# valeoai/PAFUSE

Hardware: AMD Instinct MI355X
Metric: hypotheses/sec through DDIM loop (H3WB 133-kp, P=20, T=10) (higher is better)
Workload: dtype bf16x3 (every fp32 GEMM operand as the exact sum of three bf16 slices, six bf16 MFMA products per fp32-equivalent product, fp32 accumulate; activations, LayerNorm, softmax, attention and everything in memory fp32; the residual stream stored centred on its row means)

## Files before the change

pafuse_amd/csrc/kernels.hpp:

```cpp
#pragma once
#include <hip/hip_runtime.h>
#include <stdint.h>

#include <utility>

namespace pafuse {

typedef float f32x16 __attribute__((ext_vector_type(16)));
typedef float f32x4 __attribute__((ext_vector_type(4)));

constexpr int BK = 32;
constexpr int LDK = 36;

typedef __bf16 bf16x8 __attribute__((ext_vector_type(8)));
__device__ __forceinline__ bf16x8 to_bf16x8(const f32x4 lo, const f32x4 hi) {
    bf16x8 v;
#pragma unroll
    for (int i = 0; i < 4; ++i) v[i] = (__bf16)lo[i], v[4 + i] = (__bf16)hi[i];
    return v;
}

#ifdef PAFUSE_MFMA_K8
typedef __bf16 bf16x4_t __attribute__((ext_vector_type(4)));
typedef short s16x4_t __attribute__((ext_vector_type(4)));
// ... 1254 lines not shown
                    } else {
                        asm volatile("s_waitcnt lgkmcnt(3)" : "+v"(wf[g & 1][0]), "+v"(wf[g & 1][1]), "+v"(wf[g & 1][2]));
                    }
                } else {
                    asm volatile("s_waitcnt lgkmcnt(0)" : "+v"(wf[g & 1][0]), "+v"(wf[g & 1][1]), "+v"(wf[g & 1][2]));
                }
                const u32x4(&w)[3] = wf[g & 1];
                auto mm = [&](int wi, int ai) {
                    PAFUSE_PIN_ACC(acc[nt]);
                    acc[nt] = mfma_bf16_k16(__builtin_bit_cast(bf16x8, w[wi]), __builtin_bit_cast(bf16x8, cur[ai]), acc[nt]);
                };
                auto pins = [&]() {
    #pragma unroll
                    for (int q = q0; q < q1; ++q) PAFUSE_PIN_PAIR(sp[q]);
                };
                pins();
                mm(0, 2);
                {
                    constexpr int PER = (CNT + NG - 1) / NG, j0 = g * PER, j1 = (g + 1) * PER < CNT ? (g + 1) * PER : CNT;
                    if constexpr (j0 < j1 && ABL < 2) {
                        asm volatile("" ::: "memory");
                        if (refill) {
    #pragma unroll
                            for (int j = j0; j < j1; ++j) issue_piece(kn, stn, j);
                        }
                        asm volatile("" ::: "memory");
                    }
                }
    #pragma unroll
                for (int q = q0; q < q1; ++q) sp[q].template stage<0>();
                pins();
                mm(2, 0);
    #pragma unroll
                for (int q = q0; q < q1; ++q) sp[q].template stage<1>();
                pins();
                mm(1, 1);
    #pragma unroll
                for (int q = q0; q < q1; ++q) sp[q].template stage<2>();
                pins();
                mm(0, 1);
    #pragma unroll
                for (int q = q0; q < q1; ++q) sp[q].template stage<3>();
                pins();
                mm(1, 0);
    #pragma unroll
                for (int q = q0; q < q1; ++q) {
                    sp[q].template stage<4>();
                    nxt[0][q] = sp[q].s0, nxt[1][q] = sp[q].s1, nxt[2][q] = sp[q].s2;
                }
                pins();
                mm(0, 0);
                if constexpr (g == NT - 1 && ABL < 3 && NS2 == 2) cur[0] = nxt[0], cur[1] = nxt[1], cur[2] = nxt[2];
                if constexpr (g == NT - 1 && ABL >= 3 && NS2 == 2) {
    #pragma unroll
                    for (int q = 0; q < 4; ++q)
                        cur[0][q] = cur[2][q] = __builtin_bit_cast(uint32_t, sp[q].x0), cur[1][q] = __builtin_bit_cast(uint32_t, sp[q].x1);
                }
            });
    #undef PAFUSE_PIN_ACC
    #undef PAFUSE_PIN_PAIR
            __builtin_amdgcn_s_setprio(0);
        }
    }
    PAFUSE_STAMP(1);
    __syncthreads();
    constexpr int VEC = EPI == EPI_BIAS ? 0 : (7 * BM * WN + 3) / 4 * 4;
    if constexpr (VEC > 0) {
        static_assert((size_t)(VEC + 5 * BN) * sizeof(float) <= (size_t)NSTAGE * T::STAGE_BYTES, "epilogue vectors must fit the ring");
        const float* const src[5] = {p.bias, p.post_w, p.post_b, p.next_w, p.next_b};
#pragma unroll
        for (int v = 0; v < 5; ++v)
            if (src[v])
                for (int i = tid; i < BN / 4; i += T::NTHR)
                    *reinterpret_cast<f32x4*>(smem + VEC + v * BN + 4 * i) = *reinterpret_cast<const f32x4*>(src[v] + n0 + 4 * i);
        __syncthreads();
    }
    if constexpr (ABL == 4) {
        float sacc = 0.f;
#pragma unroll
        for (int nt = 0; nt < NT; ++nt)
#pragma unroll
            for (int i = 0; i < 16; ++i) sacc += acc[nt][i];
        if (sacc == 123.456f) p.out[0] = sacc;
        return;
    }
    if constexpr (EPI == EPI_ROWLN && SLAB) {
        constexpr size_t RINGF = (size_t)NSTAGE * T::STAGE_BYTES / sizeof(float);
        constexpr auto need = [](int nth) { return (size_t)VEC + 5 * BN + (size_t)NW * 32 * (32 * nth + 4); };
        constexpr int NTH = (NT % 2 == 0 && need(2) <= RINGF) ? 2 : 1;
        static_assert(need(NTH) <= RINGF, "epilogue scratch must fit the ring");
        epilogue_rows_h<WN, NT, BM, NW, NTH, false, 2>(acc, p, m0, n0, wm, wn, r, h, wave, lane, smem, 1.0f);
    } else {
        epilogue_row_per_lane<WN, NT, BM, EPI, VEC>(acc, p, m0, n0, wm, wn, r, h, smem);
    }
}

template <int WM, int WN, int NT, int EPI, int NSTAGE, int MINW, int ABL = 0, int BKC = 32>
__global__ void __launch_bounds__(WM* WN * 64, MINW) gemm_dma_kernel(const GemmParams p) {
    PAFUSE_XQ_GUARD();
    extern __shared__ __attribute__((aligned(16))) float smem[];
    gemm_dma_tile<WM, WN, NT, EPI, NSTAGE, ABL, BKC>(p, blockIdx.x, gridDim.x, smem);
}

constexpr int GROUP_MAX = 4;
struct GroupedGemmParams {
    GemmParams p[GROUP_MAX];
    int first[GROUP_MAX + 1];
    int n;
};

template <int EPI>
__global__ void __launch_bounds__(256, 2) grouped_rowln_kernel(const GroupedGemmParams g) {
    PAFUSE_XQ_GUARD();
    extern __shared__ __attribute__((aligned(16))) float smem[];
    const int b = blockIdx.x;
    int s = 0;
#pragma unroll
    for (int i = 1; i < GROUP_MAX; ++i)
        if (i < g.n && b >= g.first[i]) s = i;
    const GemmParams& p = g.p[s];
    const int lb = b - g.first[s], nb = g.first[s + 1] - g.first[s];
    switch (p.N) {
        case 384: gemm_dma_tile<2, 2, 6, EPI, 2, 0, 16, false>(p, lb, nb, smem); break;
        case 256: gemm_dma_tile<2, 2, 4, EPI, 2, 0, 16, false>(p, lb, nb, smem); break;
        case 224: gemm_dma_tile<4, 1, 7, EPI, 2, 0, 16, false>(p, lb, nb, smem); break;
        default: break;
    }
}

struct AttnParams {
    const float* qkv;
    float* o;
    uint8_t* o_h;
    int64_t nseq;
    int L, C, heads, d;
    int64_t group, group_stride, seq_stride, tok_stride;
    float scale;
};

template <int ITEMS>
__device__ __forceinline__ void attn_item(int64_t i, int64_t nseq, int heads, int64_t& seq, int& head) {
    if (nseq % 8 == 0 && ((nseq / 8) * heads) % ITEMS == 0) {
        const int64_t blk = i / ITEMS;
        const int lo = (int)(blk % 8);
        const int64_t u = (blk / 8) * ITEMS + (i % ITEMS);
        head = (int)(u % heads);
        seq = (u / heads) * 8 + lo;
    } else {
        seq = i / heads;
        head = (int)(i % heads);
    }
}

template <int LP, int DP, int NW>
__global__ void __launch_bounds__(NW * 64) attn_kernel(const AttnParams p) {
    PAFUSE_XQ_GUARD();
    constexpr int QT = LP / 16, KT = LP / 16, CT = DP / 16, SD = DP / 16, ITEMS = NW / QT, LDV = DP + 4;
    constexpr int NTHR = NW * 64, C4 = DP / 4;
    static_assert(NW % QT == 0, "waves must be a multiple of the query tiles");
    extern __shared__ __attribute__((aligned(16))) float smem[];
    float* Ks = smem;
    float* Vs = smem + ITEMS * LP * LDV;
    const int tid = threadIdx.x, lane = tid & 63, wave = tid >> 6;
    const int64_t nitems = p.nseq * p.heads;
    const int C3 = 3 * p.C;

    const int il = wave / QT, qt = wave % QT;
    const int64_t item = (int64_t)blockIdx.x * ITEMS + il;
    const bool mine = item < nitems;
    int64_t seq = 0;
    int head = 0;
    if (mine) attn_item<ITEMS>(item, p.nseq, p.heads, seq, head);
    const int64_t base = (seq / p.group) * p.group_stride + (seq % p.group) * p.seq_stride;
    const int l15 = lane & 15, g = lane >> 4;
    f32x4 qf[SD];
    {
        const int q = qt * 16 + l15;
#pragma unroll
        for (int s = 0; s < SD; ++s) {
            qf[s] = f32x4{0.f, 0.f, 0.f, 0.f};
            if (mine && q < p.L && 16 * s + 4 * g < p.d)
                qf[s] = *reinterpret_cast<const f32x4*>(p.qkv + (base + q * p.tok_stride) * C3 + head * p.d + 16 * s +
                                                        4 * g);
        }
    }
    for (int sl = 0; sl < ITEMS; ++sl) {
        const int64_t it2 = (int64_t)blockIdx.x * ITEMS + sl;
        const bool ok = it2 < nitems;
        int64_t seq2 = 0;
        int head2 = 0;
        if (ok) attn_item<ITEMS>(it2, p.nseq, p.heads, seq2, head2);
        const int64_t base2 = (seq2 / p.group) * p.group_stride + (seq2 % p.group) * p.seq_stride;
        for (int idx = tid; idx < LP * C4; idx += NTHR) {
            const int t = idx / C4, c4 = idx % C4;
            f32x4 kv = {0.f, 0.f, 0.f, 0.f}, vv = {0.f, 0.f, 0.f, 0.f};
            if (ok && t < p.L && c4 * 4 < p.d) {
                const float* src = p.qkv + (base2 + t * p.tok_stride) * C3 + head2 * p.d + c4 * 4;
                kv = *reinterpret_cast<const f32x4*>(src + p.C);
                vv = *reinterpret_cast<const f32x4*>(src + 2 * p.C);
            }
            *reinterpret_cast<f32x4*>(Ks + (sl * LP + t) * LDV + c4 * 4) = kv;
            *reinterpret_cast<f32x4*>(Vs + (sl * LP + t) * LDV + c4 * 4) = vv;
        }
    }
    __syncthreads();
    if (!mine) return;
    const float* Kb = Ks + il * LP * LDV;
    const float* Vb = Vs + il * LP * LDV;
    f32x4 sc[KT];
#pragma unroll
    for (int kt = 0; kt < KT; ++kt) sc[kt] = f32x4{0.f, 0.f, 0.f, 0.f};
#pragma unroll
    for (int s = 0; s < SD; ++s) {
        f32x4 kf[KT];
#pragma unroll
        for (int kt = 0; kt < KT; ++kt)
            kf[kt] = *reinterpret_cast<const f32x4*>(Kb + (kt * 16 + l15) * LDV + 16 * s + 4 * g);
#pragma unroll
        for (int j = 0; j < 4; ++j)
#pragma unroll
            for (int kt = 0; kt < KT; ++kt)
                sc[kt] = __builtin_amdgcn_mfma_f32_16x16x4f32(kf[kt][j], qf[s][j], sc[kt], 0, 0, 0);
    }
    float mx = -INFINITY;
#pragma unroll
    for (int kt = 0; kt < KT; ++kt)
#pragma unroll
        for (int reg = 0; reg < 4; ++reg) {
            const int key = kt * 16 + 4 * g + reg;
            const float v = key < p.L ? sc[kt][reg] * p.scale : -INFINITY;
            sc[kt][reg] = v;
            mx = fmaxf(mx, v);
        }
    mx = fmaxf(mx, __shfl_xor(mx, 16));
    mx = fmaxf(mx, __shfl_xor(mx, 32));
    float sum = 0.f;
#pragma unroll
    for (int kt = 0; kt < KT; ++kt)
#pragma unroll
        for (int reg = 0; reg < 4; ++reg) {
            const float e = __builtin_amdgcn_exp2f((sc[kt][reg] - mx) * 1.44269504088896340736f);
            sc[kt][reg] = e;
            sum += e;
        }
    sum += __shfl_xor(sum, 16);
    sum += __shfl_xor(sum, 32);
    const float inv = 1.0f / sum;
#pragma unroll
    for (int kt = 0; kt < KT; ++kt)
#pragma unroll
        for (int reg = 0; reg < 4; ++reg) sc[kt][reg] *= inv;

    f32x4 oc[CT];
#pragma unroll
    for (int ct = 0; ct < CT; ++ct) oc[ct] = f32x4{0.f, 0.f, 0.f, 0.f};
#pragma unroll
    for (int kt = 0; kt < KT; ++kt)
#pragma unroll
        for (int reg = 0; reg < 4; ++reg) {
            const float* vrow = Vb + (kt * 16 + 4 * g + reg) * LDV + l15;
#pragma unroll
            for (int ct = 0; ct < CT; ++ct)
                oc[ct] = __builtin_amdgcn_mfma_f32_16x16x4f32(vrow[ct * 16], sc[kt][reg], oc[ct], 0, 0, 0);
        }
    const int q = qt * 16 + l15;
    if (q < p.L) {
        if (p.o_h) {
            uint8_t* const hrow = p.o_h + (base + q * p.tok_stride) * p.C * 4;
#pragma unroll
            for (int ct = 0; ct < CT; ++ct)
                if (ct * 16 + 4 * g < p.d) {
                    const int c = head * p.d + ct * 16 + 4 * g;
                    hsplit_store4(hrow + (c >> 3) * 32, c & 4, oc[ct]);
                }
            return;
        }
        float* orow = p.o + (base + q * p.tok_stride) * p.C + head * p.d + 4 * g;
#pragma unroll
        for (int ct = 0; ct < CT; ++ct)
            if (ct * 16 + 4 * g < p.d) *reinterpret_cast<f32x4*>(orow + ct * 16) = oc[ct];
    }
}

constexpr int ATTN_LONG_LP = 256;
template <int DP>
__global__ void __launch_bounds__(1024) attn_long_kernel(const AttnParams p) {
    PAFUSE_XQ_GUARD();
    constexpr int LP = ATTN_LONG_LP, T = LP / 16, SD = DP / 16, CT = DP / 16, LDV = DP + 4, C4 = DP / 4;
    extern __shared__ __attribute__((aligned(16))) float smem[];
    float* Ks = smem;
    float* Vs = smem + LP * LDV;
    const int tid = threadIdx.x, lane = tid & 63, w = tid >> 6, l15 = lane & 15, g = lane >> 4;
    int64_t seq;
    int head;
    attn_item<1>((int64_t)blockIdx.x, p.nseq, p.heads, seq, head);
    const int64_t base = (seq / p.group) * p.group_stride + (seq % p.group) * p.seq_stride;
    const int C3 = 3 * p.C, nt = (p.L + 15) / 16;
    f32x4 qf[SD];
    {
        const int q = 16 * w + l15;
#pragma unroll
        for (int s = 0; s < SD; ++s) {
            qf[s] = f32x4{0.f, 0.f, 0.f, 0.f};
            if (q < p.L && 16 * s + 4 * g < p.d)
                qf[s] = *reinterpret_cast<const f32x4*>(p.qkv + (base + (int64_t)q * p.tok_stride) * C3 + head * p.d + 16 * s + 4 * g);
        }
    }
    for (int idx = tid; idx < nt * 16 * C4; idx += 1024) {
        const int t = idx / C4, c4 = idx % C4;
        f32x4 kv = {0.f, 0.f, 0.f, 0.f}, vv = {0.f, 0.f, 0.f, 0.f};
        if (t < p.L && c4 * 4 < p.d) {
            const float* src = p.qkv + (base + (int64_t)t * p.tok_stride) * C3 + head * p.d + c4 * 4;
            kv = *reinterpret_cast<const f32x4*>(src + p.C);
            vv = *reinterpret_cast<const f32x4*>(src + 2 * p.C);
        }
        *reinterpret_cast<f32x4*>(Ks + t * LDV + c4 * 4) = kv;
        *reinterpret_cast<f32x4*>(Vs + t * LDV + c4 * 4) = vv;
    }
    __syncthreads();
    if (w >= nt) return;
    f32x4 sc[T];
#pragma unroll
    for (int kt = 0; kt < T; ++kt) {
        sc[kt] = f32x4{0.f, 0.f, 0.f, 0.f};
        if (kt < nt) {
#pragma unroll
            for (int s = 0; s < SD; ++s) {
                const f32x4 kf = *reinterpret_cast<const f32x4*>(Ks + (kt * 16 + l15) * LDV + 16 * s + 4 * g);
#pragma unroll
                for (int j = 0; j < 4; ++j) sc[kt] = __builtin_amdgcn_mfma_f32_16x16x4f32(kf[j], qf[s][j], sc[kt], 0, 0, 0);
            }
        }
    }
    float mx = -INFINITY;
#pragma unroll
    for (int kt = 0; kt < T; ++kt)
#pragma unroll
        for (int reg = 0; reg < 4; ++reg) {
            const float v = kt * 16 + 4 * g + reg < p.L ? sc[kt][reg] * p.scale : -INFINITY;
            sc[kt][reg] = v;
            mx = fmaxf(mx, v);
        }
    mx = fmaxf(mx, __shfl_xor(mx, 16));
    mx = fmaxf(mx, __shfl_xor(mx, 32));
    float sum = 0.f;
#pragma unroll
    for (int kt = 0; kt < T; ++kt)
#pragma unroll
        for (int reg = 0; reg < 4; ++reg) {
            const float e = __builtin_amdgcn_exp2f((sc[kt][reg] - mx) * 1.44269504088896340736f);
            sc[kt][reg] = e;
            sum += e;
        }
    sum += __shfl_xor(sum, 16);
    sum += __shfl_xor(sum, 32);
    const float inv = 1.0f / sum;
    f32x4 oc[CT];
#pragma unroll
    for (int ct = 0; ct < CT; ++ct) oc[ct] = f32x4{0.f, 0.f, 0.f, 0.f};
#pragma unroll
    for (int kt = 0; kt < T; ++kt)
        if (kt < nt) {
#pragma unroll
            for (int reg = 0; reg < 4; ++reg) {
                const float pr = sc[kt][reg] * inv;
                const float* vrow = Vs + (kt * 16 + 4 * g + reg) * LDV + l15;
#pragma unroll
                for (int ct = 0; ct < CT; ++ct) oc[ct] = __builtin_amdgcn_mfma_f32_16x16x4f32(vrow[ct * 16], pr, oc[ct], 0, 0, 0);
            }
        }
    const int q = 16 * w + l15;
    if (q < p.L) {
        float* orow = p.o + (base + (int64_t)q * p.tok_stride) * p.C + head * p.d + 4 * g;
#pragma unroll
        for (int ct = 0; ct < CT; ++ct)
            if (ct * 16 + 4 * g < p.d) *reinterpret_cast<f32x4*>(orow + ct * 16) = oc[ct];
    }
}

struct FqaParams {
    GemmParams g;
    float* o;
    int64_t nseq;
    int L, C, heads, d, nseq_tile;
    int64_t group, group_stride, seq_stride, tok_stride;
    float scale;
};

template <int LP, int DP>
struct FqaTile {
    static constexpr int NB = 3 * DP / 16, LDV = DP + 4, ROWS = 128 + (LP == 48 ? 4 : 0);
    static constexpr int STAGE_BYTES = Tile16<NB>::STAGE_BYTES, QKV_BYTES = 3 * ROWS * LDV * 4;
    static constexpr int LDS_BYTES = STAGE_BYTES > QKV_BYTES ? STAGE_BYTES : QKV_BYTES;
};

template <int LP, int DP>
__global__ void __launch_bounds__(256, 2) fqa_kernel(const FqaParams fp) {
    PAFUSE_XQ_GUARD();
    using FT = FqaTile<LP, DP>;
    constexpr int NB = FT::NB, LDV = FT::LDV, ROWS = FT::ROWS;
    using T = Tile16<NB>;
    constexpr int A_LD = T::A_LD, W_LD = T::W_LD, NTHR = T::NTHR;
    extern __shared__ __attribute__((aligned(16))) float smem[];
    const GemmParams& p = fp.g;
    uint8_t* const As = reinterpret_cast<uint8_t*>(smem);
    uint8_t* const Ws = As + T::A_BYTES;
    const int tid = threadIdx.x, lane = tid & 63, wave = tid >> 6;
    const int c = lane & 15, qd = lane >> 4;
    const int L = fp.L, NSEQ = fp.nseq_tile;
    const int64_t ntiles = (fp.nseq + NSEQ - 1) / NSEQ;
    const int xcd = blockIdx.x & 7, idx = blockIdx.x >> 3;
    const int64_t tile = (int64_t)(idx / fp.heads) * 8 + xcd;
    const int head = idx % fp.heads;
    if (tile >= ntiles) return;
    const int K = p.K, nk = K / 32;
    const int64_t seq0 = tile * NSEQ;
    const int64_t last_seq = fp.nseq - 1;
    auto token_of = [&](int r) -> int64_t {
        int sl = r / L, t = r - sl * L;
        if (sl >= NSEQ) sl = NSEQ - 1, t = L - 1;
        int64_t sq = seq0 + sl;
        if (sq > last_seq) sq = last_seq;
        return (sq / fp.group) * fp.group_stride + (sq % fp.group) * fp.seq_stride + t * fp.tok_stride;
    };

    const float* a_ptr[A_LD];
    int a_dst[A_LD];
#pragma unroll
    for (int i = 0; i < A_LD; ++i) {
        const int g = 2 * wave + (i >> 1), j = 4 * (i & 1) + qd;
        a_ptr[i] = p.A + token_of(16 * g + c) * K + 4 * j;
        a_dst[i] = g * 2048 + (j & 1) * 1024 + ((j >> 1) * 16 + c) * 16;
    }
// ... 3246 lines not shown
```

pafuse_amd/csrc/pafuse_hip.hip:

```cpp
#include "../../include/pafuse_hip.h"

#include <hip/hip_runtime.h>

#include <algorithm>
#include <cmath>
#include <cstdarg>
#include <cstdio>
#include <cstdlib>
#include <cstring>
#include <type_traits>

#include "kernels.hpp"
#include "hgemm.hpp"
#include "xgemm.hpp"
#include "sgemm.hpp"
#include "train_kernels.hpp"

using namespace pafuse;

namespace {

thread_local char g_err[512] = "";

int fail(int code, const char* fmt, ...) {
// ... 372 lines not shown
        if (p.N % 64 == 0) return launch_gemm<4, 1, 2, EPI_BIAS, 1, 4, 0, 2>(p, s);
    }
    if (p.M <= 0) return PAFUSE_OK;
    if (p.K % BK || p.N % 32 || p.K <= 0 || p.N <= 0)
        return fail(PAFUSE_E_SHAPE, "linear: N=%d K=%d must be positive multiples of 32", p.N, p.K);
    if ((p.out_act || p.dact_u) && ((p.N % 64 && !(p.mode == MODE_BF16X3 && p.wlayout == WLAYOUT_M16)) || mode_images(p.mode) || p.ln_in || p.act))
        return fail(PAFUSE_E_ARG, "linear: out_act / dact_u need N %% 64 == 0 and a plain fp32 or bf16x3 product");
    if (p.mode == MODE_F16X2) return hgemm_bias(p, s);
    if (p.mode == MODE_BF16X3_IMAGES) return xgemm_bias(p, s);
#ifdef PAFUSE_QKV_32X32
    p.wlayout = WLAYOUT_PLAIN;
#endif
#ifndef PAFUSE_NO_STRIP
    if (strip2_ok(p)) return strip2_bias(p, s);
#endif
    if (p.mode == MODE_BF16X3 && p.wlayout == WLAYOUT_M16) {
        if (p.N % 128 == 0) return launch_gemm16<8, 3>(p, s);
        if (p.N % 96 == 0) return launch_gemm16<6, 3>(p, s);
        if (p.N % 112 == 0) return launch_gemm16<7, 3>(p, s);
        if (p.N % 64 == 0) return launch_gemm16<4, 4>(p, s);
        return launch_gemm16<2, 4>(p, s);
    }
    if (p.mode == MODE_BF16X3) {
        if (p.N % 128 == 0 && p.M >= 4096) return launch_gemm<4, 1, 4, EPI_BIAS, 1, PAFUSE_FC1_MINW, 0, 2>(p, s);
        if (p.N % 64 == 0) return launch_gemm<4, 1, 2, EPI_BIAS, 1, 4, 0, 2>(p, s);
        if (p.N % 96 == 0) return launch_gemm<4, 1, 3, EPI_BIAS, 1, 1, 1, 2>(p, s);
        return launch_gemm<4, 1, 1, EPI_BIAS, 1, 1, 0, 2>(p, s);
    }
    if (p.mode != MODE_F32) {
        if (p.N % 64 == 0) return launch_gemm<4, 1, 2, EPI_BIAS, 1, 5, 0, 1>(p, s);
        if (p.N % 96 == 0) return launch_gemm<4, 1, 3, EPI_BIAS, 1, 1, 1, 1>(p, s);
        return launch_gemm<4, 1, 1, EPI_BIAS, 1, 1, 0, 1>(p, s);
    }
    if (p.N % 64 == 0) return launch_gemm<4, 1, 2, EPI_BIAS, 1, 5>(p, s);
    if (p.N % 96 == 0) return launch_gemm<4, 1, 3, EPI_BIAS, 1, 1, 1>(p, s);
    return launch_gemm<4, 1, 1, EPI_BIAS, 1>(p, s);
}

template <int EPI>
int gemm_rowln_as(const GemmParams& p0, hipStream_t s) {
    GemmParams p = p0;
    if (p.mode == MODE_BF16X3 && (debug_f32_mask() & 2)) p.mode = MODE_F32;
    if (p.M <= 0) return PAFUSE_OK;
    if (p.K % BK || p.K <= 0) return fail(PAFUSE_E_SHAPE, "rowln: K=%d must be a positive multiple of 32", p.K);
    if (p.mode == MODE_F16X2 || p.mode == MODE_BF16X3_IMAGES) {
        if constexpr (EPI == EPI_ROWLN) return p.mode == MODE_F16X2 ? hgemm_rowln(p, s) : xgemm_rowln(p, s);
        else return fail(PAFUSE_E_ARG, "training has no image-pipeline kernels");
    }
    if constexpr (EPI == EPI_ROWLN_TRAIN) {
        if (p.mode == MODE_BF16X3) {
            switch (p.N) {
                case 384: return launch_gemm_dma<2, 2, 6, EPI, 2, 2, 16>(p, s);
                case 256: return launch_gemm_dma<2, 2, 4, EPI, 2, 2, 16>(p, s);
                case 224: if (p.M >= 4096) return launch_gemm_dma<4, 1, 7, EPI, 2, 2, 16>(p, s); break;
                default: break;
            }
            p.mode = MODE_F32;
        }
    }
    if constexpr (EPI == EPI_ROWLN) {
        if (p.mode == MODE_BF16X3) {
            switch (p.N) {
                case 384: return launch_gemm_dma<2, 2, 6, EPI, 2, 2, 16>(p, s);
                case 256: return launch_gemm_dma<2, 2, 4, EPI, 2, 2, 16>(p, s);
                case 288: return launch_gemm_dma<2, 3, 3, EPI, 2, 2, 16>(p, s);
                case 224:
                    return p.M >= 4096 ? launch_gemm_dma<4, 1, 7, EPI, 2, 2, 16>(p, s) : launch_gemm_dma<2, 1, 7, EPI, 2, 2, 16>(p, s);
                case 128: return launch_gemm<1, 4, 1, EPI, 1, 1, 1, 2>(p, s);
                case 64: return launch_gemm<1, 2, 1, EPI, 1, 1, 1, 2>(p, s);
                default: break;
            }
        } else if (p.mode != MODE_F32) {
            switch (p.N) {
                case 384: return launch_gemm<1, 4, 3, EPI, 1, 1, 1, 1>(p, s);
                case 288: return launch_gemm<1, 3, 3, EPI, 1, 1, 1, 1>(p, s);
                case 256: return launch_gemm<2, 2, 4, EPI, 1, 2, 1, 1>(p, s);
                case 224: return launch_gemm<1, 7, 1, EPI, 1, 1, 1, 1>(p, s);
                case 128: return launch_gemm<1, 4, 1, EPI, 1, 1, 1, 1>(p, s);
                case 64: return launch_gemm<1, 2, 1, EPI, 1, 1, 1, 1>(p, s);
                default: break;
            }
        }
    }
    switch (p.N) {
        case 384: return launch_gemm<1, 4, 3, EPI, 1, 1, 1>(p, s);
        case 288: return launch_gemm<1, 3, 3, EPI, 1, 1, 1>(p, s);
        case 256: return launch_gemm<2, 2, 4, EPI, 1, 2, 1>(p, s);
        case 224: return launch_gemm<1, 7, 1, EPI, 1, 1, 1>(p, s);
        case 128: return launch_gemm<1, 4, 1, EPI, 1, 1, 1>(p, s);
        case 64: return launch_gemm<1, 2, 1, EPI, 1, 1, 1>(p, s);
        default: return fail(PAFUSE_E_SHAPE, "no whole-row kernel for channel width %d (have 64,128,224,256,288,384)", p.N);
    }
}

int gemm_rowln(const GemmParams& p, hipStream_t s) { return gemm_rowln_as<EPI_ROWLN>(p, s); }
int gemm_rowln_train(const GemmParams& p, hipStream_t s) { return gemm_rowln_as<EPI_ROWLN_TRAIN>(p, s); }

bool group_ok_rowln(const GemmParams& p) {
    return p.mode == MODE_BF16X3 && p.Wsplit && (p.N == 384 || p.N == 256 || (p.N == 224 && p.M >= 4096)) && p.K % 16 == 0 && p.K > 0 &&
           !(debug_f32_mask() & 2);
}

template <bool ROWLN>
int gemm_group(const GemmParams* ps, int n, hipStream_t s, bool shared_grids) {
    bool ok = ROWLN && shared_grids && n >= 2 && n <= GROUP_MAX;
    for (int i = 0; i < n && ok; ++i) ok = ps[i].M > 0 && group_ok_rowln(ps[i]);
    if (!ok) {
        for (int i = 0; i < n; ++i) {
            const int rc = ROWLN ? gemm_rowln(ps[i], s) : gemm_bias(ps[i], s);
            if (rc) return rc;
        }
        return PAFUSE_OK;
    }
    int order[GROUP_MAX];
    double cost[GROUP_MAX];
    int64_t tiles[GROUP_MAX];
    for (int i = 0; i < n; ++i) {
        const GemmParams& p = ps[i];
        int bm, bn;
        bm = p.N == 224 ? 128 : 64, bn = p.N;
        tiles[i] = (p.M + bm - 1) / bm * (p.N / bn);
        cost[i] = (double)bm * bn * p.K;
        order[i] = i;
    }
    std::sort(order, order + n, [&](int a, int b) { return cost[a] > cost[b]; });
    GroupedGemmParams g{};
    g.n = n;
    int64_t first = 0;
    for (int k = 0; k < n; ++k) {
        g.p[k] = ps[order[k]];
        g.first[k] = (int)first;
        first += (tiles[order[k]] + 7) / 8 * 8;
        if (first > 0x7fffffff) return fail(PAFUSE_E_ARG, "grouped gemm grid out of range");
    }
    g.first[n] = (int)first;
    for (int k = n + 1; k <= GROUP_MAX; ++k) g.first[k] = (int)first;
    constexpr size_t lds = 2 * DmaTile<2, 2, 6, 16>::STAGE_BYTES;
    static_assert(lds >= 2 * DmaTile<2, 2, 4, 16>::STAGE_BYTES && lds >= 2 * DmaTile<4, 1, 7, 16>::STAGE_BYTES && lds <= 80 * 1024, "LDS");
    return launch<grouped_rowln_kernel<EPI_ROWLN>>("grouped_rowln_kernel", (unsigned)first, 256, lds, s, g);
}

bool width_supported(int C) { return C == 384 || C == 288 || C == 256 || C == 224 || C == 128 || C == 64; }

template <int LP, int DP, int NW>
int launch_attn(const AttnParams& p, hipStream_t s) {
    constexpr int ITEMS = NW / (LP / 16);
    constexpr size_t lds = (size_t)2 * ITEMS * LP * (DP + 4) * sizeof(float);
    const int64_t nitems = p.nseq * p.heads;
    const int64_t grid = (nitems + ITEMS - 1) / ITEMS;
    if (grid > 0x7fffffff) return fail(PAFUSE_E_ARG, "attention grid out of range");
    return launch<attn_kernel<LP, DP, NW>>("attn_kernel", (unsigned)grid, NW * 64, lds, s, p);
}

template <int DP>
int launch_attn_long(const AttnParams& p, hipStream_t s) {
    constexpr size_t lds = (size_t)2 * ATTN_LONG_LP * (DP + 4) * sizeof(float);
    static_assert(lds <= 160 * 1024, "LDS");
    const int64_t grid = p.nseq * p.heads;
    if (grid > 0x7fffffff) return fail(PAFUSE_E_ARG, "attention grid out of range");
    return launch<attn_long_kernel<DP>>("attn_long_kernel", (unsigned)grid, 1024, lds, s, p);
}

int attention(const AttnParams& p, hipStream_t s) {
    if (p.nseq <= 0) return PAFUSE_OK;
#ifdef PAFUSE_ABL_NO_ATTENTION
    return PAFUSE_OK;
#endif
    if (p.d % 4 || p.d > 48 || p.L > ATTN_LONG_LP || p.L <= 0)
        return fail(PAFUSE_E_SHAPE, "attention: head dim %d (need %%4, <=48) / length %d (need <=%d)", p.d, p.L, ATTN_LONG_LP);
    if (p.L > 144) {
        if (p.o_h) return fail(PAFUSE_E_SHAPE, "attention: no f16x2 image output for sequences of %d > 144 tokens: use mode 2", p.L);
        return p.d <= 32 ? launch_attn_long<32>(p, s) : launch_attn_long<48>(p, s);
    }
    const int dp = p.d <= 32 ? 32 : 48;
    const int lp = p.L <= 32 ? 32 : (p.L <= 48 ? 48 : (p.L <= 80 ? 80 : 144));
    if (lp == 144)
        return dp == 32 ? launch_attn<144, 32, 9>(p, s) : launch_attn<144, 48, 9>(p, s);
    if (dp == 32) {
        if (lp == 32) return launch_attn<32, 32, 4>(p, s);
        if (lp == 48) return launch_attn<48, 32, 6>(p, s);
        return launch_attn<80, 32, 5>(p, s);
    }
    if (lp == 32) return launch_attn<32, 48, 4>(p, s);
    if (lp == 48) return launch_attn<48, 48, 6>(p, s);
    return launch_attn<80, 48, 5>(p, s);
}

constexpr size_t RANGE_FLAG_BYTES = 256;

struct PartBuffers {
    float *x, *xn, *o, *wide;
    int eb;
    float* temb;
    float* pred;
    float* stats;
};

size_t part_buffer_bytes(int64_t M, int C, int B, int eb = 4) {
    return align_up((size_t)M * C * 4) + 2 * align_up((size_t)M * C * eb) + align_up((size_t)M * 3 * C * 4) + align_up((size_t)B * C * 4) +
           align_up((size_t)M * 3 * 4) + align_up((size_t)M * 2 * 4);
}

char* carve_part(char* base, int64_t M, int C, int B, PartBuffers& pb, int eb = 4) {
    pb.eb = eb;
    pb.x = (float*)base;
    base += align_up((size_t)M * C * 4);
    pb.xn = (float*)base;
    base += align_up((size_t)M * C * eb);
    pb.o = (float*)base;
    base += align_up((size_t)M * C * eb);
    pb.wide = (float*)base;
    base += align_up((size_t)M * 3 * C * 4);
    pb.temb = (float*)base;
    base += align_up((size_t)B * C * 4);
    pb.pred = (float*)base;
    base += align_up((size_t)M * 3 * 4);
    pb.stats = (float*)base;
    base += align_up((size_t)M * 2 * 4);
    return base;
}

PartBuffers offset_rows(const PartBuffers& pb, int64_t row0, int C) {
    PartBuffers o = pb;
    const int64_t img = row0 * C * pb.eb / 4;
    o.x = pb.x + row0 * C, o.xn = pb.xn + img, o.o = pb.o + img, o.wide = pb.wide + row0 * 3 * C;
    o.pred = pb.pred + row0 * 3;
    o.stats = pb.stats + row0 * 2;
    return o;
}

static bool ln_folded(const pafuse_mixste2_weights* w) { return w->ste[0].qkv_lt != nullptr; }
static bool h_residual_only(const pafuse_mixste2_weights* w) { return mode_images(w->operand_bf16) && ln_folded(w) && !w->keep_f32_residual; }

static void embed_outputs(EmbedParams& e, int mode, bool folded, bool h_only, float* x, float* xn, void* image, float* stats,
                          int64_t row0, int64_t nrows) {
    e.x = h_only ? nullptr : x, e.xn = xn;
    e.stats = folded ? stats : nullptr;
    e.xh = mode_images(mode) ? reinterpret_cast<uint8_t*>(image) : nullptr;
    e.x_image = mode == MODE_BF16X3_IMAGES;
    e.centre_x = mode == MODE_BF16X3 && folded;
    e.row0 = row0, e.nrows = nrows;
}

int check_weights(const pafuse_mixste2_weights* w, bool training = false) {
    if (!w) return fail(PAFUSE_E_ARG, "null weights");
    static_assert(EMBED_NV * 128 >= 384, "embed kernel covers the widest part");
    if (w->in_chans != 5) return fail(PAFUSE_E_SHAPE, "in_chans must be 5, got %d", w->in_chans);
    if (w->depth < 1 || w->depth > PAFUSE_MAX_DEPTH) return fail(PAFUSE_E_SHAPE, "depth %d out of range", w->depth);
    if (!width_supported(w->channels)) return fail(PAFUSE_E_SHAPE, "channel width %d has no kernel", w->channels);
    if (w->heads <= 0 || w->channels % w->heads) return fail(PAFUSE_E_SHAPE, "heads %d !| C %d", w->heads, w->channels);
    const int d = w->channels / w->heads;
    if (d % 4 || d > 48) return fail(PAFUSE_E_SHAPE, "head dim %d unsupported", d);
    if (w->joints < 1 || w->joints > 144 || w->frames < 1 || w->frames > ATTN_LONG_LP)
        return fail(PAFUSE_E_SHAPE, "sequence lengths J=%d F=%d: J must be in 1..144, F in 1..%d", w->joints, w->frames, ATTN_LONG_LP);
    if (w->operand_bf16 == MODE_F16X2 && w->frames > 144)
        return fail(PAFUSE_E_SHAPE, "f16x2: no attention form for clips of %d > 144 frames: use mode 2", w->frames);
    if (!mode_valid(w->operand_bf16)) return fail(PAFUSE_E_ARG, "matrix-product mode %d", w->operand_bf16);
    if (mode_images(w->operand_bf16)) {
        const int hidden = w->mlp_hidden > 0 ? w->mlp_hidden : 2 * w->channels;
        if (!hgemm_width(w->channels) || !hgemm_plain_n(3 * w->channels) || !hgemm_plain_n(hidden) || hidden % 32)
            return fail(PAFUSE_E_SHAPE, "the image pipelines (f16x2, bf16x3 on images) serve the widths 224 / 256 / 384 with an MLP hidden "
                                        "width that is a multiple of 128 or 224 (got C = %d, hidden = %d): use mode 2", w->channels, hidden);
    }
    if (w->operand_bf16 == MODE_BF16X3_IMAGES && !training) {
        for (int i = 0; i < w->depth; ++i)
            for (const pafuse_block_weights* b : {&w->ste[i], &w->tte[i]})
                if (!b->qkv_hs || !b->qkv_hb) return fail(PAFUSE_E_ARG, "bf16x3 on images needs the head-major qkv image of every block (qkv_hs, qkv_hb)");
        if (!xfqa_has(w->joints, d, w->heads) || !xfqa_has(w->frames, d, w->heads))
            return fail(PAFUSE_E_SHAPE, "bf16x3 on images: no fused qkv + attention form for sequences of %d / %d tokens at head dim %d, %d heads: "
                                        "use mode 2", w->joints, w->frames, d, w->heads);
    }
    if (w->mlp_hidden < 0 || (w->mlp_hidden > 0 && (w->mlp_hidden % 32 || w->mlp_hidden > 3 * w->channels)))
        return fail(PAFUSE_E_SHAPE, "mlp hidden width %d must be a multiple of 32 and at most 3C = %d", w->mlp_hidden, 3 * w->channels);
    if (!(w->qk_scale >= 0.f)) return fail(PAFUSE_E_ARG, "qk_scale must be positive (0 = head_dim^-0.5)");
    if (training && (w->operand_bf16 == MODE_BF16 || mode_images(w->operand_bf16)))
        return fail(PAFUSE_E_ARG, "training runs fp32 ('f32') or split-precision ('bf16x3') products");
    if (mode_split(w->operand_bf16) && !training)
        for (int i = 0; i < w->depth; ++i)
            for (const pafuse_block_weights* b : {&w->ste[i], &w->tte[i]})
                if ((!b->qkv_ws && w->operand_bf16 != MODE_BF16X3_IMAGES) || !b->proj_ws || !b->fc1_ws || !b->fc2_ws)
                    return fail(PAFUSE_E_ARG, "split-precision mode needs the pre-split image of every linear weight "
                                              "(pafuse_split_weights)");
    const bool fold = ln_folded(w);
    for (int i = 0; i < w->depth; ++i)
        for (const pafuse_block_weights* b : {&w->ste[i], &w->tte[i]}) {
            const int set = (b->qkv_lt != nullptr) + (b->fc1_lt != nullptr);
            if (set != (fold ? 2 : 0)) return fail(PAFUSE_E_ARG, "folded-LayerNorm vectors (qkv_lt, fc1_lt) must be set in every block or in none");
        }
    if (fold && !mode_split(w->operand_bf16)) return fail(PAFUSE_E_ARG, "the folded LayerNorm exists in the split-precision modes only");
    return PAFUSE_OK;
}

struct BlockTail {
    const float *post_w, *post_b;
    float post_eps;
    const float* pos;
    int posJ, posF;
    const float *next_w, *next_b;
    float next_eps;
    const float *head_w, *head_b;
    float* out_head;
};

struct BlockLaunch {
    GemmParams qkv, proj, fc1, fc2;
    AttnParams attn;
    FqaParams fqa;
    bool fused;
    MlpParams mlp;
    bool mlp_fused;
};

BlockLaunch make_block(const pafuse_block_weights& bw, const PartBuffers& pb, int64_t M, int C, int heads, int64_t nseq, int L,
                       int64_t group, int64_t group_stride, int64_t seq_stride, int64_t tok_stride, const BlockTail& tail,
                       int mode, int hidden = 0, float qk_scale = 0.f, bool fold = false, bool keep_f32_residual = false) {
    if (hidden <= 0) hidden = 2 * C;
    BlockLaunch b{};
    float* const stats = pb.stats;
    const bool hp = mode_images(mode);
    uint8_t* const xn_h = reinterpret_cast<uint8_t*>(pb.xn);
    const bool h_residual = hp && fold && !keep_f32_residual;
    GemmParams& g = b.qkv;
    g.A = pb.xn, g.W = bw.qkv_w, g.bias = bw.qkv_b, g.out = pb.wide, g.M = M, g.N = 3 * C, g.K = C, g.act = 0;
    g.mode = mode, g.Wsplit = (const uint8_t*)bw.qkv_ws, g.wlayout = WLAYOUT_M16;
    if (fold) g.A = pb.x, g.ln_in = stats, g.bias = bw.qkv_lt;
    if (hp) g.Ah = xn_h, g.Wh = (const uint8_t*)bw.qkv_ws;
    if (fold) g.ln_s = nullptr;
    AttnParams& a = b.attn;
    a.qkv = pb.wide, a.o = pb.o, a.nseq = nseq, a.L = L, a.C = C, a.heads = heads, a.d = C / heads;
    a.group = group, a.group_stride = group_stride, a.seq_stride = seq_stride, a.tok_stride = tok_stride;
    a.scale = qk_scale != 0.f ? qk_scale : 1.0f / sqrtf((float)(C / heads));
    if (hp) a.o_h = reinterpret_cast<uint8_t*>(pb.o);
    b.fused = false;
    if (mode_split(mode) && bw.qkv_hs && bw.qkv_hb && (mode == MODE_BF16X3_IMAGES ? xfqa_has(L, C / heads, heads) : fqa_has(L, C / heads, mode))) {
        const int lp = fqa_lp(L, mode), dp = fqa_dp(C / heads);
        FqaParams& f = b.fqa;
        f.g = g;
// ... 2041 lines not shown
```

Before: 107.1.

## Add one-wave-per-item attention kernel with register-held K and block-free sync

Factors the score/softmax/PV tile into a shared helper and adds an attention kernel in which each wave owns a whole (sequence, head) item. The wave keeps K fragments in registers, stages only V in wave-private LDS, and loops over query tiles while prefetching the next Q fragment. This drops block-wide __syncthreads and LDS staging of K, and lets the launch-bounds hint trade registers for occupancy. The dispatcher routes several mid-length shapes to the new kernel. Holding K in registers risks register pressure and spilling for the longer tiles.

```diff
diff --git a/pafuse_amd/csrc/kernels.hpp b/pafuse_amd/csrc/kernels.hpp
--- a/pafuse_amd/csrc/kernels.hpp
+++ b/pafuse_amd/csrc/kernels.hpp
@@ -1430,6 +1430,83 @@
     }
 }
 
+template <int KT, int SD, int CT, int LDV, class KFrag>
+__device__ __forceinline__ void attn_tile(const AttnParams& p, const f32x4 (&qf)[SD], KFrag&& kfrag, const float* Vb, int qt,
+                                          int64_t base, int head, int l15, int g) {
+    f32x4 sc[KT];
+#pragma unroll
+    for (int kt = 0; kt < KT; ++kt) sc[kt] = f32x4{0.f, 0.f, 0.f, 0.f};
+#pragma unroll
+    for (int s = 0; s < SD; ++s) {
+        f32x4 kf[KT];
+#pragma unroll
+        for (int kt = 0; kt < KT; ++kt) kf[kt] = kfrag(kt, s);
+#pragma unroll
+        for (int j = 0; j < 4; ++j)
+#pragma unroll
+            for (int kt = 0; kt < KT; ++kt)
+                sc[kt] = __builtin_amdgcn_mfma_f32_16x16x4f32(kf[kt][j], qf[s][j], sc[kt], 0, 0, 0);
+    }
+    float mx = -INFINITY;
+#pragma unroll
+    for (int kt = 0; kt < KT; ++kt)
+#pragma unroll
+        for (int reg = 0; reg < 4; ++reg) {
+            const int key = kt * 16 + 4 * g + reg;
+            const float v = key < p.L ? sc[kt][reg] * p.scale : -INFINITY;
+            sc[kt][reg] = v;
+            mx = fmaxf(mx, v);
+        }
+    mx = fmaxf(mx, __shfl_xor(mx, 16));
+    mx = fmaxf(mx, __shfl_xor(mx, 32));
+    float sum = 0.f;
+#pragma unroll
+    for (int kt = 0; kt < KT; ++kt)
+#pragma unroll
+        for (int reg = 0; reg < 4; ++reg) {
+            const float e = __builtin_amdgcn_exp2f((sc[kt][reg] - mx) * 1.44269504088896340736f);
+            sc[kt][reg] = e;
+            sum += e;
+        }
+    sum += __shfl_xor(sum, 16);
+    sum += __shfl_xor(sum, 32);
+    const float inv = 1.0f / sum;
+#pragma unroll
+    for (int kt = 0; kt < KT; ++kt)
+#pragma unroll
+        for (int reg = 0; reg < 4; ++reg) sc[kt][reg] *= inv;
+
+    f32x4 oc[CT];
+#pragma unroll
+    for (int ct = 0; ct < CT; ++ct) oc[ct] = f32x4{0.f, 0.f, 0.f, 0.f};
+#pragma unroll
+    for (int kt = 0; kt < KT; ++kt)
+#pragma unroll
+        for (int reg = 0; reg < 4; ++reg) {
+            const float* vrow = Vb + (kt * 16 + 4 * g + reg) * LDV + l15;
+#pragma unroll
+            for (int ct = 0; ct < CT; ++ct)
+                oc[ct] = __builtin_amdgcn_mfma_f32_16x16x4f32(vrow[ct * 16], sc[kt][reg], oc[ct], 0, 0, 0);
+        }
+    const int q = qt * 16 + l15;
+    if (q < p.L) {
+        if (p.o_h) {
+            uint8_t* const hrow = p.o_h + (base + q * p.tok_stride) * p.C * 4;
+#pragma unroll
+            for (int ct = 0; ct < CT; ++ct)
+                if (ct * 16 + 4 * g < p.d) {
+                    const int c = head * p.d + ct * 16 + 4 * g;
+                    hsplit_store4(hrow + (c >> 3) * 32, c & 4, oc[ct]);
+                }
+            return;
+        }
+        float* orow = p.o + (base + q * p.tok_stride) * p.C + head * p.d + 4 * g;
+#pragma unroll
+        for (int ct = 0; ct < CT; ++ct)
+            if (ct * 16 + 4 * g < p.d) *reinterpret_cast<f32x4*>(orow + ct * 16) = oc[ct];
+    }
+}
+
 template <int LP, int DP, int NW>
 __global__ void __launch_bounds__(NW * 64) attn_kernel(const AttnParams p) {
     PAFUSE_XQ_GUARD();
@@ -1484,79 +1561,62 @@
     __syncthreads();
     if (!mine) return;
     const float* Kb = Ks + il * LP * LDV;
-    const float* Vb = Vs + il * LP * LDV;
-    f32x4 sc[KT];
-#pragma unroll
-    for (int kt = 0; kt < KT; ++kt) sc[kt] = f32x4{0.f, 0.f, 0.f, 0.f};
-#pragma unroll
-    for (int s = 0; s < SD; ++s) {
-        f32x4 kf[KT];
-#pragma unroll
-        for (int kt = 0; kt < KT; ++kt)
-            kf[kt] = *reinterpret_cast<const f32x4*>(Kb + (kt * 16 + l15) * LDV + 16 * s + 4 * g);
-#pragma unroll
-        for (int j = 0; j < 4; ++j)
-#pragma unroll
-            for (int kt = 0; kt < KT; ++kt)
-                sc[kt] = __builtin_amdgcn_mfma_f32_16x16x4f32(kf[kt][j], qf[s][j], sc[kt], 0, 0, 0);
-    }
-    float mx = -INFINITY;
-#pragma unroll
-    for (int kt = 0; kt < KT; ++kt)
-#pragma unroll
-        for (int reg = 0; reg < 4; ++reg) {
-            const int key = kt * 16 + 4 * g + reg;
-            const float v = key < p.L ? sc[kt][reg] * p.scale : -INFINITY;
-            sc[kt][reg] = v;
-            mx = fmaxf(mx, v);
-        }
-    mx = fmaxf(mx, __shfl_xor(mx, 16));
-    mx = fmaxf(mx, __shfl_xor(mx, 32));
-    float sum = 0.f;
-#pragma unroll
-    for (int kt = 0; kt < KT; ++kt)
-#pragma unroll
-        for (int reg = 0; reg < 4; ++reg) {
-            const float e = __builtin_amdgcn_exp2f((sc[kt][reg] - mx) * 1.44269504088896340736f);
-            sc[kt][reg] = e;
-            sum += e;
-        }
-    sum += __shfl_xor(sum, 16);
-    sum += __shfl_xor(sum, 32);
-    const float inv = 1.0f / sum;
-#pragma unroll
-    for (int kt = 0; kt < KT; ++kt)
-#pragma unroll
-        for (int reg = 0; reg < 4; ++reg) sc[kt][reg] *= inv;
-
-    f32x4 oc[CT];
-#pragma unroll
-    for (int ct = 0; ct < CT; ++ct) oc[ct] = f32x4{0.f, 0.f, 0.f, 0.f};
-#pragma unroll
-    for (int kt = 0; kt < KT; ++kt)
-#pragma unroll
-        for (int reg = 0; reg < 4; ++reg) {
-            const float* vrow = Vb + (kt * 16 + 4 * g + reg) * LDV + l15;
-#pragma unroll
-            for (int ct = 0; ct < CT; ++ct)
-                oc[ct] = __builtin_amdgcn_mfma_f32_16x16x4f32(vrow[ct * 16], sc[kt][reg], oc[ct], 0, 0, 0);
-        }
-    const int q = qt * 16 + l15;
-    if (q < p.L) {
-        if (p.o_h) {
-            uint8_t* const hrow = p.o_h + (base + q * p.tok_stride) * p.C * 4;
-#pragma unroll
-            for (int ct = 0; ct < CT; ++ct)
-                if (ct * 16 + 4 * g < p.d) {
-                    const int c = head * p.d + ct * 16 + 4 * g;
-                    hsplit_store4(hrow + (c >> 3) * 32, c & 4, oc[ct]);
-                }
-            return;
-        }
-        float* orow = p.o + (base + q * p.tok_stride) * p.C + head * p.d + 4 * g;
-#pragma unroll
-        for (int ct = 0; ct < CT; ++ct)
-            if (ct * 16 + 4 * g < p.d) *reinterpret_cast<f32x4*>(orow + ct * 16) = oc[ct];
+    attn_tile<KT, SD, CT, LDV>(
+        p, qf, [&](int kt, int s) { return *reinterpret_cast<const f32x4*>(Kb + (kt * 16 + l15) * LDV + 16 * s + 4 * g); },
+        Vs + il * LP * LDV, qt, base, head, l15, g);
+}
+
+constexpr int attn_wave_min_waves(int LP, int DP, int WPB) {
+    const int by_lds = (160 * 1024 / (WPB * LP * (DP + 4) * 4) * WPB + 3) / 4, by_regs = LP == 80 ? 3 : 4;
+    return by_lds < by_regs ? by_lds : by_regs;
+}
+template <int LP, int DP, int WPB>
+__global__ void __launch_bounds__(WPB * 64, attn_wave_min_waves(LP, DP, WPB)) attn_wave_kernel(const AttnParams p) {
+    PAFUSE_XQ_GUARD();
+    constexpr int QT = LP / 16, KT = LP / 16, CT = DP / 16, SD = DP / 16, LDV = DP + 4, C4 = DP / 4, VN = LP * C4 / 64;
+    static_assert(LP * C4 % 64 == 0, "V rows are loaded by whole waves");
+    extern __shared__ __attribute__((aligned(16))) float smem[];
+    const int lane = threadIdx.x & 63, wave = threadIdx.x >> 6, l15 = lane & 15, g = lane >> 4;
+    const int64_t item = (int64_t)blockIdx.x * WPB + wave;
+    if (item >= p.nseq * p.heads) return;
+    int64_t seq;
+    int head;
+    attn_item<WPB>(item, p.nseq, p.heads, seq, head);
+    const int64_t base = (seq / p.group) * p.group_stride + (seq % p.group) * p.seq_stride;
+    const int C3 = 3 * p.C;
+    const float* const qh = p.qkv + head * p.d;
+    float* const Vs = smem + wave * LP * LDV;
+
+    auto frag = [&](int t, int off, f32x4(&f)[SD]) {
+        const int tok = t * 16 + l15;
+#pragma unroll
+        for (int s = 0; s < SD; ++s) {
+            f[s] = f32x4{0.f, 0.f, 0.f, 0.f};
+            if (tok < p.L && 16 * s + 4 * g < p.d)
+                f[s] = *reinterpret_cast<const f32x4*>(qh + (base + tok * p.tok_stride) * C3 + off + 16 * s + 4 * g);
+        }
+    };
+    f32x4 qf[2][SD], kf[KT][SD], vv[VN];
+    frag(0, 0, qf[0]);
+#pragma unroll
+    for (int kt = 0; kt < KT; ++kt) frag(kt, p.C, kf[kt]);
+#pragma unroll
+    for (int i = 0; i < VN; ++i) {
+        const int t = (lane + 64 * i) / C4, c4 = (lane + 64 * i) % C4;
+        vv[i] = f32x4{0.f, 0.f, 0.f, 0.f};
+        if (t < p.L && c4 * 4 < p.d) vv[i] = *reinterpret_cast<const f32x4*>(qh + (base + t * p.tok_stride) * C3 + 2 * p.C + c4 * 4);
+    }
+#pragma unroll
+    for (int i = 0; i < VN; ++i) {
+        const int t = (lane + 64 * i) / C4, c4 = (lane + 64 * i) % C4;
+        *reinterpret_cast<f32x4*>(Vs + t * LDV + c4 * 4) = vv[i];
+    }
+    asm volatile("s_waitcnt lgkmcnt(0)" ::: "memory");
+#pragma unroll
+    for (int t = 0; t < QT; ++t) {
+        if (16 * t >= p.L) break;
+        if (t + 1 < QT) frag(t + 1, 0, qf[(t + 1) & 1]);
+        attn_tile<KT, SD, CT, LDV>(p, qf[t & 1], [&](int kt, int s) { return kf[kt][s]; }, Vs, t, base, head, l15, g);
     }
 }
 
diff --git a/pafuse_amd/csrc/pafuse_hip.hip b/pafuse_amd/csrc/pafuse_hip.hip
--- a/pafuse_amd/csrc/pafuse_hip.hip
+++ b/pafuse_amd/csrc/pafuse_hip.hip
@@ -548,6 +548,16 @@
     return launch<attn_kernel<LP, DP, NW>>("attn_kernel", (unsigned)grid, NW * 64, lds, s, p);
 }
 
+template <int LP, int DP, int WPB>
+int launch_attn_wave(const AttnParams& p, hipStream_t s) {
+    constexpr size_t lds = (size_t)WPB * LP * (DP + 4) * sizeof(float);
+    static_assert(lds <= 64 * 1024 && (160 * 1024 / lds) * WPB >= 12, "LDS");
+    const int64_t nitems = p.nseq * p.heads;
+    const int64_t grid = (nitems + WPB - 1) / WPB;
+    if (grid > 0x7fffffff) return fail(PAFUSE_E_ARG, "attention grid out of range");
+    return launch<attn_wave_kernel<LP, DP, WPB>>("attn_wave_kernel", (unsigned)grid, WPB * 64, lds, s, p);
+}
+
 template <int DP>
 int launch_attn_long(const AttnParams& p, hipStream_t s) {
     constexpr size_t lds = (size_t)2 * ATTN_LONG_LP * (DP + 4) * sizeof(float);
@@ -574,11 +584,11 @@
         return dp == 32 ? launch_attn<144, 32, 9>(p, s) : launch_attn<144, 48, 9>(p, s);
     if (dp == 32) {
         if (lp == 32) return launch_attn<32, 32, 4>(p, s);
-        if (lp == 48) return launch_attn<48, 32, 6>(p, s);
-        return launch_attn<80, 32, 5>(p, s);
-    }
-    if (lp == 32) return launch_attn<32, 48, 4>(p, s);
-    if (lp == 48) return launch_attn<48, 48, 6>(p, s);
+        if (lp == 48) return launch_attn_wave<48, 32, 4>(p, s);
+        return launch_attn_wave<80, 32, 4>(p, s);
+    }
+    if (lp == 32) return launch_attn_wave<32, 48, 4>(p, s);
+    if (lp == 48) return launch_attn_wave<48, 48, 4>(p, s);
     return launch_attn<80, 48, 5>(p, s);
 }
 
```

Measured after the change: 108.4, median of 6. +1.2%, better.
